# ch4r10t33r/zigz

Hardware: AMD Instinct MI355X
Metric: trace steps/sec proved (BabyBear, 2^20 RV64I trace) (higher is better)
Workload: dtype u32

## Files before the change

### zigz_amd/csrc/api_commit.cpp

```cpp
#include "api_internal.hpp"

using namespace zk;

static void caps_for(zigz_ctx *ctx, size_t npad, unsigned rn, unsigned gn) {
    ListCaps &c = ctx->caps;
    if (c.npad == npad && c.rn == rn && c.gn == gn) return;
    c.npad = npad;
    c.rn = rn;
    c.gn = gn;
    c.g_slabs = false;
    c.g_drops = c.g_skip = c.g_kept = 0;
    memset(c.r_last, 0, sizeof(c.r_last));
    memset(c.g_last, 0, sizeof(c.g_last));
    c.last_dropped = false;
    const LevelLists rw = runs_lists(npad, rn ? rn : 1), gw = cons_lists(npad);
    for (unsigned l = 0; l < RUN_MAX_LEVELS; l++) {
        c.r[l] = l <= rw.top ? (rw.cap[l] / 8 > 256 ? rw.cap[l] / 8 : 256) : 0;
        c.g[l] = l <= gw.top ? 256 : 0;
    }
}

zigz_status build_trees(zigz_ctx *ctx, const uint32_t *d_vals, size_t val_stride, size_t n_values, size_t npad,
                               uint8_t *d_slab, size_t ncols, bool record, TreeRef *ref) {
    const unsigned height = log2_floor(npad);
// ... 165 lines not shown
            if (keep) CHK(ws_get(ctx, WS_CONSMETA, kept + (upper_here ? upper_bytes : 0), &mw));
            else mw = (uint8_t *)w + ((key_bytes + idx_bytes + list_bytes + 64 + 63) & ~(size_t)63);
            b.g_rep = (uint32_t *)mw;
            t.g_rep = b.g_rep;
            t.g_store = (uint8_t *)mw + 2 * npad * 4;
            if (upper_here) t.upper = (uint8_t *)mw + kept;
            if (ctx->cons_table != w || ctx->cons_table_bytes != ctx->ws_bytes[WS_CONS] || ctx->cons_gen + RUN_MAX_LEVELS + 1 >= 4096) {
                HIPCHK(ctx, hipMemsetAsync(w, 0, key_bytes, ctx->stream));
                ctx->cons_table = w;
                ctx->cons_table_bytes = ctx->ws_bytes[WS_CONS];
                ctx->cons_gen = 1;
            }
            b.g_gen = ctx->cons_gen;
            ctx->cons_gen += top + 1;
            b.g_ctr = g_ctr;
            b.g_has_slabs = whole || ctx->caps.g_slabs;
            static const bool always_probe = getenv("ZIGZ_CONS_PROBE_ALWAYS") != nullptr;
            b.g_no_probe = ref && ctx->caps.npad == npad && ctx->caps.g_kept >= 2 && !ctx->cons_always && !always_probe;
            t.g_ncols = G.n;
            t.g_dropped = g_ctr + 8;
            for (unsigned k = 0; k < G.n; k++) t.g_j_of_col[G.c[k]] = (signed char)k;
            if (virt)
                for (unsigned k = 0; k < GS.n; k++) t.g_sd_mask |= 1ull << GS.c[k];
            ctx->build_cons_hinted = G.n;
            ctx->build_cons_levels_nodes = level_nodes;
            ctx->build_cons_sd = GS.n;
        }
        if (!t.upper) {
            void *u;
            CHK(ws_get(ctx, WS_OUT64, upper_bytes, &u));
            t.upper = (uint8_t *)u;
        }
        b.t = t;
        if (ctx->debug_skip != 2) {
            launch_runs_structure(b, ctx->stream, R.n ? stamp(4, 0) : nullptr);
            launch_cons_structure(b, ctx->stream, G.n ? stamp(4, 0) : nullptr);
        }
        if (GS.n && b.g_has_slabs) {
            const ColMap gs = slab_map(GS);
            launch_keccak_small_l01(d_vals, val_stride, n_values, npad, t.slab, stride, GS, ctx->d_sd_tables, ctx->d_sd_fallbacks + 1,
                                    (uint32_t *)sd_todo + sd_todo_words(npad, H.n), ctx->stream, stamp(3, 0), !virt, g_ctr + 8,
                                    &gs);
        }
    }
    if (ref) *ref = t;
    unsigned first_top = 0;
    if (lists) {
        for (unsigned l = 0; l <= top; l++) {
            size_t expect = 0;
            if (ref && ctx->caps.npad == npad && (ctx->caps.r_last[l] || ctx->caps.g_last[l])) {
                auto more = [](unsigned v) { return (size_t)RUN_SUBS * (v + v / 4 + 8); };
                expect = (R.n ? more(ctx->caps.r_last[l]) : 0) + (G.n ? more(ctx->caps.g_last[l]) * G.n : 0) +
                         (G.n && ctx->caps.last_dropped ? (size_t)G.n * (npad >> l) : 0);
            }
            if (ctx->debug_skip != 1) launch_level_hash(b, l, ctx->stream, stamp(5, 0), expect);
            if (l == top) break;
            ColMap m{};
            for (size_t c = 0; c < ncols; c++) {
                const int kd = kind(c);
                if (kd == 0 || (kd == 1 && l >= 1)) m.c[m.n++] = (uint8_t)c;
            }
            if (m.n) {
                const ColMap ms = slab_map(m);
                launch_keccak_level(t.slab, stride, tree_level_offset(npad, l), tree_level_offset(npad, l + 1), npad >> (l + 1), ncols,
                                    ctx->stream, stamp(keccak_level_is_wide(npad >> (l + 1), m.n) ? 1 : 2, (uint64_t)m.n * (npad >> (l + 1))), &ms);
            }
        }
        first_top = top;
    } else {
        for (unsigned l = 0; l < height; l++) {
            const size_t n_out = npad >> (l + 1);
            first_top = l;
            if (n_out <= 256) break;
            ColMap m{};
            const ColMap *pm = nullptr;
            size_t nc = ncols;
            if (H.n && l < 1) {
                for (size_t c = 0; c < ncols; c++)
                    if (kind(c) == 0) m.c[m.n++] = (uint8_t)c;
                if (m.n == 0) continue;
                pm = &m;
                nc = m.n;
            }
            launch_keccak_level(t.slab, stride, tree_level_offset(npad, l), tree_level_offset(npad, l + 1), n_out, ncols, ctx->stream,
                                stamp(keccak_level_is_wide(n_out, nc) ? 1 : 2, (uint64_t)nc * n_out), pm);
        }
    }
    if (height) {
// ... 321 lines not shown
    b.rcols = R;
    b.gcols = G;
    if (R.n) {
        t.bitmap = (unsigned long long *)(a0 + o_bitmap);
        t.prev = (unsigned short *)(a0 + o_prev);
        t.woff = (unsigned short *)(a0 + o_woff);
        t.ubase = (uint32_t *)(a0 + o_ubase);
        t.r_store = a0 + o_rstore;
        b.r_list = (uint32_t *)(a0 + o_rlist);
        b.r_stage = a0 + o_rstage;
        b.r_ctr = (unsigned long long *)(a0 + o_rctr);
    }
    if (G.n) {
        t.slab = a0 + o_slab;
        t.g_rep = (const uint32_t *)(a0 + o_grep);
        t.g_store = a0 + o_gstore;
        t.g_dropped = (const unsigned long long *)(a0 + o_gctr) + 8;
        b.g_keys = (unsigned long long *)(a0 + o_keys);
        b.g_idx = (uint32_t *)(a0 + o_idx);
        b.g_list = (uint32_t *)(a0 + o_glist);
        b.g_rep = (uint32_t *)(a0 + o_grep);
        b.g_ctr = (unsigned long long *)(a0 + o_gctr);
        b.g_has_slabs = 1;
        b.g_gen = ctx->batch_gen;
        ctx->batch_gen += t.top + 1;
    }
    b.t = t;
    set_zstride(b, S, nz);
    t = b.t;
    ColSrcs cs{};
    for (unsigned z = 0; z < nz; z++) cs.p[z] = srcs[z];
    launch_gather_cols(cs, nz, nc, N, src_stride, (uint32_t *)(a0 + o_cols), stride, S, ctx->stream);
    launch_zero_counters(nullptr, R.n ? b.r_ctr : nullptr, G.n ? b.g_ctr : nullptr, ctx->stream, nz, S);
    if (ctx->debug_skip != 2) {
        launch_runs_structure(b, ctx->stream, nullptr);
        launch_cons_structure(b, ctx->stream, nullptr);
    }
    for (unsigned l = 0; l <= t.top; l++)
        if (ctx->debug_skip != 1) launch_level_hash(b, l, ctx->stream, nullptr);
    if (height && ctx->debug_skip != 1) launch_merkle_top(t, t.top, height, nc, ctx->stream, nullptr);
    HIPCHK(ctx, hipGetLastError());
    job->tree = t;
    job->d_cols = (const uint32_t *)(a0 + o_cols);
    job->col_stride = stride;
    job->zstride = S;
    job->off_r_ctr = o_rctr;
    job->off_g_ctr = o_gctr;
    job->whole = false;
    const DoneFlag done = done_flag(ctx, 0);
    job->roots_seq = done.seq;
    launch_job_summary(t, height, ctx->h_roots, nc, R.n ? b.r_ctr : nullptr, nullptr, G.n ? b.g_ctr : nullptr, ctx->stream, done);
    HIPCHK(ctx, hipGetLastError());
    HIPCHK(ctx, hipEventRecord(job->built, ctx->stream));
    uint64_t level_nodes = 0;
    for (unsigned l = 0; l <= t.top; l++) level_nodes += npad >> l;
    job->run_cols = R.n;
    job->run_dense = (uint64_t)R.n * level_nodes;
    job->sd_cols = 0;
    job->cons_hinted = G.n;
    job->cons_levels_nodes = level_nodes;
    job->cons_sd = 0;
    job->perms0 = (uint64_t)nc * (2 * N - 1);
    job->no_eval_skip = ctx->debug_skip == 2;
    return ZIGZ_OK;
}

extern "C" zigz_status zigz_commit_begin_batch(zigz_ctx *ctx, const uint32_t *const *d_cols, size_t nproofs, size_t ncols,
                                               size_t col_stride, size_t nv, zigz_commit_job **out) {
    ZIGZ_ENTER(ctx);
    if (!ctx || !d_cols || !out || ncols == 0 || nproofs == 0 || nproofs > BATCH_MAX || nv > 40) return ZIGZ_ERR_INVALID_ARGUMENT;
    if (ncols * nproofs > ROOTS_MAX_COLS || col_stride < ((size_t)1 << nv)) return ZIGZ_ERR_INVALID_ARGUMENT;
    for (size_t z = 0; z < nproofs; z++)
// ... 302 lines not shown
```

### zigz_amd/csrc/kernels.hpp

```cpp
#pragma once
#include <hip/hip_runtime.h>
#include <stddef.h>
#include <stdint.h>

namespace zk {

struct KTime {
    hipEvent_t start, stop;
};

inline size_t tree_level_offset(size_t npad, unsigned level) { return 2 * npad - 2 * (npad >> level); }
inline size_t tree_nodes(size_t npad) { return 2 * npad; }

void launch_narrow_u64(const uint64_t *d_in, uint32_t *d_out, size_t n, uint32_t *d_flag, hipStream_t s);
void launch_reduce_u64(const uint64_t *d_in, uint32_t *d_out, size_t n, hipStream_t s);
void launch_witness_rows(const uint64_t *d_rows, size_t num_steps, size_t npad, uint32_t *d_cols, size_t stride,
                         hipStream_t s);
void launch_widen_u32(const uint32_t *d_in, uint64_t *d_out, size_t n, hipStream_t s);
struct TraceStep {
    uint64_t pc, rd_value, mem_addr, mem_value;
    int64_t imm;
    uint8_t opcode, rd, rs1, rs2, funct3, funct7, wr_reg, mem_is_read;
};
static_assert(sizeof(TraceStep) == 48, "TraceStep must mirror zigz_trace_step (48 bytes)");
// ... 155 lines not shown
LevelLists runs_lists(size_t npad, size_t ncols, const unsigned *cap_in = nullptr);
LevelLists cons_lists(size_t npad, const unsigned *cap_in = nullptr);
size_t runs_units(size_t npad, size_t ncols, unsigned long long ubase_off[RUN_MAX_LEVELS]);
size_t runs_stage_scratch_bytes(size_t npad, size_t ncols);

struct MerkleBuild {
    ZPtr<const uint32_t> vals;
    size_t val_stride, n_values, npad;
    TreeRef t;
    ColMap rcols;
    ZPtr<uint32_t> r_list;
    ZPtr<unsigned long long> r_ctr;
    ZPtr<uint8_t> r_stage;
    ColMap gcols;
    ColMap gcols_sd;
    int g_has_slabs;
    int g_no_probe;
    ZPtr<unsigned long long> g_keys;
    ZPtr<uint32_t> g_idx;
    ZPtr<uint32_t> g_rep;
    ZPtr<uint32_t> g_list;
    ZPtr<unsigned long long> g_ctr;
    unsigned g_gen;
};
inline void set_zstride(MerkleBuild &b, size_t zs, unsigned nz) {
    TreeRef &t = b.t;
    t.zstride = zs;
    t.nz = nz;
    t.slab.zs = t.upper.zs = t.bitmap.zs = t.prev.zs = t.woff.zs = t.ubase.zs = t.r_store.zs = t.g_rep.zs = t.g_store.zs = t.g_dropped.zs = zs;
    b.vals.zs = b.r_list.zs = b.r_ctr.zs = b.r_stage.zs = b.g_keys.zs = b.g_idx.zs = b.g_rep.zs = b.g_list.zs = b.g_ctr.zs = zs;
}
void launch_runs_structure(const MerkleBuild &b, hipStream_t s, const KTime *kt = nullptr);
void launch_cons_structure(const MerkleBuild &b, hipStream_t s, const KTime *kt = nullptr);
void launch_level_hash(const MerkleBuild &b, unsigned L, hipStream_t s, const KTime *kt = nullptr, size_t expect = 0);
void launch_fill_virtual(const MerkleBuild &b, hipStream_t s);
void launch_merkle_top(const TreeRef &t, unsigned first_level, unsigned height, size_t ncols, hipStream_t s, const KTime *kt = nullptr);
void launch_keccak_leaves(const uint32_t *d_vals, size_t val_stride, size_t n_values, size_t npad,
                          uint8_t *d_tree, size_t tree_stride_nodes, size_t ncols, hipStream_t s, const KTime *kt = nullptr,
                          const ColMap *cols = nullptr, const ColMap *slabs = nullptr);
void launch_keccak_level(uint8_t *d_tree, size_t tree_stride_nodes, size_t in_off, size_t out_off, size_t n_out,
                         size_t ncols, hipStream_t s, const KTime *kt = nullptr, const ColMap *slabs = nullptr);
constexpr unsigned SD_DOMAIN = 128;
constexpr size_t SD_TABLE_BYTES = (size_t)(SD_DOMAIN + SD_DOMAIN * SD_DOMAIN) * 32;
void launch_sd_tables(uint8_t *d_tables, hipStream_t s);
inline size_t sd_todo_words(size_t npad, size_t ncols) { return 2 * ncols * ((npad / 2 + 63) / 64) + 2; }
void launch_keccak_small_l01(const uint32_t *d_vals, size_t val_stride, size_t n_values, size_t npad, uint8_t *d_tree,
                             size_t tree_stride_nodes, const ColMap &cols, const uint8_t *d_tables,
                             unsigned long long *d_todo_count, uint32_t *d_todo, hipStream_t s, const KTime *kt = nullptr,
                             bool write_leaves = true, const unsigned long long *d_only_if = nullptr,
                             const ColMap *slabs = nullptr);
bool keccak_level_is_wide(size_t n_out, size_t ncols);
struct DoneFlag {
    unsigned *count = nullptr;
    unsigned long long *flag = nullptr;
    unsigned long long seq = 0;
};
void launch_publish_u64(unsigned long long *d_src, size_t n, unsigned long long *h_dst, bool rezero, hipStream_t s, DoneFlag done);
void launch_publish_u32(const uint32_t *d_src, size_t n, uint32_t *h_dst, hipStream_t s, DoneFlag done);
void launch_paths(const TreeRef &t, size_t n_values, unsigned height, const uint32_t *d_vals, size_t val_stride,
                  const uint64_t *d_idx, uint8_t *d_sib, uint8_t *d_dirs, uint32_t *d_leaf, size_t ncols, hipStream_t s,
                  DoneFlag done = DoneFlag());
TreeRef slab_tree_ref(uint8_t *d_tree, size_t npad);
void launch_gather_nodes(const uint8_t *d_tree, size_t tree_stride_nodes, size_t node, uint8_t *d_out, size_t ncols,
                         hipStream_t s);
constexpr unsigned JOB_SUMMARY_WORDS = 8 + 2 * RUN_MAX_LEVELS;
void launch_zero_counters(unsigned long long *d_sd_ctr, unsigned long long *d_r_ctr, unsigned long long *d_g_ctr, hipStream_t s,
                          unsigned nz = 0, size_t zstride = 0);
// ... 109 lines not shown
```

### zigz_amd/csrc/merkle_levels.hip

```cpp
#include "kernels.hpp"
#include "tree_dev.hpp"

namespace zk {

#ifndef ZK_CONS_TPB
#define ZK_CONS_TPB 256
#endif
constexpr int CONS_TPB = ZK_CONS_TPB;

static unsigned log2u(size_t n) { unsigned l = 0; while (((size_t)1 << l) < n) l++; return l; }

static size_t stage_fv_bytes(size_t npad, size_t ncols, unsigned s) { return ncols * (npad >> (s * RUN_STAGE_LEVELS)) * 4; }
static size_t stage_inner_bytes(size_t npad, size_t ncols, unsigned s) {
    const size_t n = npad >> (s * RUN_STAGE_LEVELS);
    return ncols * ((n + 63) / 64) * 8;
}
static size_t stage_off(size_t npad, size_t ncols, unsigned s) {
    size_t off = 0;
    for (unsigned t = 1; t < s; t++) off += stage_fv_bytes(npad, ncols, t) + stage_inner_bytes(npad, ncols, t);
    return off;
}
size_t runs_stage_scratch_bytes(size_t npad, size_t ncols) {
    const unsigned top = run_top_level(npad);
    size_t b = 64;
// ... 57 lines not shown
    x = (x | (x >> 1)) & 0x3333333333333333ull;
    x = (x | (x >> 2)) & 0x0f0f0f0f0f0f0f0full;
    x = (x | (x >> 4)) & 0x00ff00ff00ff00ffull;
    x = (x | (x >> 8)) & 0x0000ffff0000ffffull;
    x = (x | (x >> 16)) & 0x00000000ffffffffull;
    return x;
}

template <int CTRL, int ROW_MASK, int BANK_MASK>
__device__ __forceinline__ int dpp_i32(int old, int v) { return __builtin_amdgcn_update_dpp(old, v, CTRL, ROW_MASK, BANK_MASK, false); }
__device__ __forceinline__ unsigned wave_scan_add(unsigned v) {
    int s = (int)v;
    s += dpp_i32<0x111, 0xf, 0xf>(0, s);
    s += dpp_i32<0x112, 0xf, 0xf>(0, s);
    s += dpp_i32<0x114, 0xf, 0xf>(0, s);
    s += dpp_i32<0x118, 0xf, 0xf>(0, s);
    s += dpp_i32<0x142, 0xa, 0xf>(0, s);
    s += dpp_i32<0x143, 0xc, 0xf>(0, s);
    return (unsigned)s;
}
__device__ __forceinline__ int wave_scan_max(int v) {
    int s = v, t;
    t = dpp_i32<0x111, 0xf, 0xf>(-1, s); s = s > t ? s : t;
    t = dpp_i32<0x112, 0xf, 0xf>(-1, s); s = s > t ? s : t;
    t = dpp_i32<0x114, 0xf, 0xf>(-1, s); s = s > t ? s : t;
    t = dpp_i32<0x118, 0xf, 0xf>(-1, s); s = s > t ? s : t;
    t = dpp_i32<0x142, 0xa, 0xf>(-1, s); s = s > t ? s : t;
    t = dpp_i32<0x143, 0xc, 0xf>(-1, s); s = s > t ? s : t;
    return s;
}

constexpr int RUNS_WAVES = TPB / 64;
template <bool STAGE0>
__global__ __launch_bounds__(TPB) void k_runs_stage(MerkleBuild b, unsigned stage, unsigned seg_log2, unsigned rmax, unsigned nseg,
                                                    size_t in_off , size_t out_off ) {
    ZK_PRIO_SMALL();
    const unsigned lane = threadIdx.x & 63, wave = threadIdx.x >> 6;
    const unsigned y = blockIdx.y, segi = blockIdx.x * RUNS_WAVES + wave;
    if (segi >= nseg) return;
    const unsigned seg = 1u << seg_log2, words = seg / 64;
    const unsigned l_in = stage * RUN_STAGE_LEVELS;
    const size_t n_in = b.npad >> l_in;
    const size_t first = (size_t)segi * seg;
    unsigned long long E = 0, I = 0;
    uint32_t fv_mine = 0;
    {
        const uint32_t *src;
        size_t limit;
        if (STAGE0) {
            src = b.vals + (size_t)b.rcols.c[y] * b.val_stride + first;
            limit = b.n_values > first ? b.n_values - first : 0;
        } else {
            src = reinterpret_cast<const uint32_t *>(b.r_stage + in_off) + (size_t)y * n_in + first;
            limit = seg;
            const unsigned long long *inner = reinterpret_cast<const unsigned long long *>(
                b.r_stage + in_off + (size_t)b.rcols.n * n_in * 4) + ((size_t)y * n_in + first) / 64;
            if (lane < words) I = inner[lane];
        }
        uint32_t prev_last = 0;
        for (unsigned q0 = 0; q0 < words; q0 += 32) {
            uint32_t x[32];
#pragma unroll
            for (unsigned j = 0; j < 32; j++) {
                const unsigned i = (q0 + j) * 64 + lane;
                x[j] = (q0 + j < words && i < limit) ? src[i] : 0u;
            }
#pragma unroll
            for (unsigned j = 0; j < 32; j++) {
                const unsigned q = q0 + j;
                uint32_t left = (uint32_t)__builtin_amdgcn_update_dpp(0, (int)x[j], 0x138 , 0xf, 0xf, false);
                if (lane == 0) left = prev_last;
// ... 60 lines not shown
                                    ((size_t)y * n_out) / 64 + segi;
        fv[lane] = fv_mine;
        if (lane == 0) *inner = I;
    }
    unsigned my_slot = 0, my_room = 0;
    if (lane <= rmax && (STAGE0 || lane != 0)) {
        const unsigned l_abs = l_in + lane;
        const unsigned sub = (y * nseg + segi) % RUN_SUBS;
        const unsigned cap = b.t.r_lists.cap[l_abs];
        const unsigned long long pos = atomicAdd(&b.r_ctr[run_ctr_index(l_abs, sub)], (unsigned long long)my_tot);
        if (pos + my_tot > cap) atomicOr(&b.r_ctr[10], 1ull);
        my_room = pos >= cap ? 0u : (unsigned)(cap - pos < my_tot ? cap - pos : my_tot);
        my_slot = sub * cap + (unsigned)(pos < cap ? pos : cap);
        b.t.ubase[b.t.ubase_off[l_abs] + (size_t)y * nseg + segi] = my_slot;
    }
#pragma unroll
    for (unsigned r = 0; r <= RUN_STAGE_LEVELS; r++) {
        if (r > rmax || (!STAGE0 && r == 0)) continue;
        const unsigned slot0 = __shfl(my_slot, r), room = __shfl(my_room, r);
        uint32_t *list = b.r_list + b.t.r_lists.base[l_in + r];
        const size_t node0 = first >> r;
        const unsigned wr = words >> r;
        for (unsigned q = 0; q < wr; q++) {
            const unsigned lo = (unsigned)__builtin_amdgcn_readlane((int)(unsigned)need_r[r], q);
            const unsigned hi = (unsigned)__builtin_amdgcn_readlane((int)(unsigned)(need_r[r] >> 32), q);
            if ((lo | hi) == 0) continue;
            const unsigned o = (unsigned)__builtin_amdgcn_readlane((int)off_r[r], q);
            const unsigned long long m = ((unsigned long long)hi << 32) | lo;
            const unsigned at = o + __builtin_amdgcn_mbcnt_hi(hi, __builtin_amdgcn_mbcnt_lo(lo, 0));
            if (((m >> lane) & 1) && at < room) list[slot0 + at] = ((uint32_t)y << RUN_NODE_BITS) | (uint32_t)(node0 + q * 64 + lane);
        }
    }
}

void launch_runs_structure(const MerkleBuild &b, hipStream_t s, const KTime *kt) {
    if (b.rcols.n == 0) return;
    const unsigned top = b.t.r_lists.top;
    unsigned nstages = 1;
    while (nstages * RUN_STAGE_LEVELS < top) nstages++;
    for (unsigned st = 0; st < nstages; st++) {
        const size_t n_in = b.npad >> (st * RUN_STAGE_LEVELS);
        const size_t seg = n_in < RUN_SEG ? n_in : RUN_SEG;
        const unsigned rmax = top - st * RUN_STAGE_LEVELS < RUN_STAGE_LEVELS ? top - st * RUN_STAGE_LEVELS : RUN_STAGE_LEVELS;
        const bool has_next = st + 1 < nstages;
        const size_t in_off = st ? stage_off(b.npad, b.rcols.n, st) : 0;
        const size_t out_off = has_next ? stage_off(b.npad, b.rcols.n, st + 1) : ~(size_t)0;
        const unsigned nseg = (unsigned)(n_in / seg);
        const dim3 grid((nseg + RUNS_WAVES - 1) / RUNS_WAVES, b.rcols.n, b.t.nz ? b.t.nz : 1);
        hipEvent_t e0 = kt && st == 0 ? kt->start : nullptr, e1 = kt && st + 1 == nstages ? kt->stop : nullptr;
        if (st == 0) {
            if (e0 || e1) hipExtLaunchKernelGGL(k_runs_stage<true>, grid, dim3(TPB), 0, s, e0, e1, 0, b, st, log2u(seg), rmax, nseg, in_off, out_off);
            else hipLaunchKernelGGL(k_runs_stage<true>, grid, dim3(TPB), 0, s, b, st, log2u(seg), rmax, nseg, in_off, out_off);
        } else {
            if (e0 || e1) hipExtLaunchKernelGGL(k_runs_stage<false>, grid, dim3(TPB), 0, s, e0, e1, 0, b, st, log2u(seg), rmax, nseg, in_off, out_off);
            else hipLaunchKernelGGL(k_runs_stage<false>, grid, dim3(TPB), 0, s, b, st, log2u(seg), rmax, nseg, in_off, out_off);
        }
    }
}

constexpr unsigned CONS_GEN_SHIFT = 52;
__device__ __forceinline__ unsigned long long cons_mix(unsigned long long x) {
    x ^= x >> 30; x *= 0xbf58476d1ce4e5b9ull;
    x ^= x >> 27; x *= 0x94d049bb133111ebull;
    return x ^ (x >> 31);
}
constexpr unsigned CONS_TUP = 16;
__device__ __forceinline__ unsigned long long cons_leaf_payload(const MerkleBuild &b, size_t k, uint32_t *tup = nullptr) {
    unsigned long long h = 0x243f6a8885a308d3ull;
    if (tup && b.gcols.n <= CONS_TUP) {
#pragma unroll
        for (unsigned j = 0; j < CONS_TUP; j++) {
            tup[j] = (j < b.gcols.n && k < b.n_values) ? b.vals[(size_t)b.gcols.c[j] * b.val_stride + k] : 0u;
            if (j < b.gcols.n) h = cons_mix(h ^ tup[j]);
        }
    } else {
        for (unsigned j = 0; j < b.gcols.n; j++)
            h = cons_mix(h ^ (k < b.n_values ? b.vals[(size_t)b.gcols.c[j] * b.val_stride + k] : 0u));
    }
    return h & ((1ull << CONS_GEN_SHIFT) - 1);
}
__device__ __forceinline__ unsigned wave_leader(unsigned long long key, bool valid, unsigned lane) {
    unsigned long long pend = __ballot(valid);
    unsigned mine = lane;
    while (pend) {
        const unsigned ld = (unsigned)__builtin_ctzll(pend);
        const unsigned long long kk = __shfl(key, ld);
        const bool same = valid && key == kk;
        if (same) mine = ld;
// ... 39 lines not shown
}
__device__ __forceinline__ uint32_t cons_lookup(const unsigned long long *keys, const uint32_t *idx, size_t mask, unsigned long long key) {
    size_t slot = cons_mix(key) & mask;
    for (size_t tries = 0; tries <= mask; tries++) {
        if (keys[slot] == key) return idx[slot];
        slot = (slot + 1) & mask;
    }
    return 0xffffffffu;
}
constexpr unsigned CONS_SET = 2 * CONS_TPB;
__device__ __forceinline__ bool wg_first(unsigned long long *set, unsigned long long key) {
    unsigned slot = (unsigned)(cons_mix(key) >> 40) & (CONS_SET - 1);
    for (;;) {
        const unsigned long long old = atomicCAS(&set[slot], 0ull, key);
        if (old == 0) return true;
        if (old == key) return false;
        slot = (slot + 1) & (CONS_SET - 1);
    }
}
__device__ __forceinline__ void cons_insert_level(const MerkleBuild &b, unsigned long long *s_set, unsigned l, unsigned long long key,
                                                  bool elected, uint32_t node, unsigned lane, size_t wave_global) {
    const size_t mask = 2 * b.npad - 1;
    size_t where = 0;
    const unsigned g = b.g_gen + l;
    const bool won = elected && wg_first(s_set, key) && cons_insert(b.g_keys, mask, key, g, l ? g - 1 : g, &where);
    const unsigned slot = cons_take_slot(b, l, won, lane, wave_global);
    if (won) {
        b.g_list[b.t.g_lists.base[l] + slot] = node;
        b.g_idx[where] = slot;
    }
}

constexpr unsigned CONS_SAMPLE = 16;
__global__ __launch_bounds__(CONS_TPB) void k_cons_leaf_insert(MerkleBuild b, int sample) {
    ZK_PRIO_SMALL();
    __shared__ unsigned long long s_set[CONS_SET];
    if (!sample && b.g_ctr[8]) return;
    for (unsigned i = threadIdx.x; i < CONS_SET; i += CONS_TPB) s_set[i] = 0;
    __syncthreads();
    const size_t k = (size_t)blockIdx.x * CONS_TPB + threadIdx.x;
    if (sample && ((k / 64) % CONS_SAMPLE) != 0) return;
    const unsigned lane = threadIdx.x & 63;
    const bool valid = k < b.npad;
    const unsigned long long key = ((unsigned long long)b.g_gen << CONS_GEN_SHIFT) | (valid ? cons_leaf_payload(b, k) : 0);
    const unsigned ld = wave_leader(key, valid, lane);
    cons_insert_level(b, s_set, 0, key, valid && ld == lane, (uint32_t)k, lane, k / 64);
}

template <bool LEAF>
__global__ __launch_bounds__(CONS_TPB) void k_cons_pass(MerkleBuild b, unsigned lr, int do_insert) {
    ZK_PRIO_SMALL();
    __shared__ unsigned long long s_set[CONS_SET];
    if (b.g_ctr[8]) return;
    for (unsigned i = threadIdx.x; i < CONS_SET; i += CONS_TPB) s_set[i] = 0;
    __syncthreads();
    const size_t n = b.npad >> lr, c = (size_t)blockIdx.x * CONS_TPB + threadIdx.x;
    const unsigned lane = threadIdx.x & 63;
    const bool valid = c < n;
    const size_t mask = 2 * b.npad - 1;
    const unsigned g_r = b.g_gen + lr;
    const size_t off = 2 * b.npad - 2 * n;
    const size_t off_in = LEAF ? 0 : 2 * b.npad - 2 * (b.npad >> (lr - 1));
    unsigned long long key = (unsigned long long)g_r << CONS_GEN_SHIFT;
    uint32_t tup[CONS_TUP];
    if (valid) {
        if (LEAF) key |= cons_leaf_payload(b, c, tup);
        else {
            const uint2 p = *reinterpret_cast<const uint2 *>(b.g_rep + off_in + 2 * c);
            key |= ((unsigned long long)p.x << RUN_NODE_BITS) | p.y;
        }
    }
    const unsigned ld = wave_leader(key, valid, lane);
    uint32_t r = 0xffffffffu;
    if (valid && ld == lane) r = cons_lookup(b.g_keys, b.g_idx, mask, key);
    r = __shfl(r, ld);
    bool alone = false;
    if (LEAF && valid && r != 0xffffffffu) {
        const size_t rn = b.g_list[b.t.g_lists.base[0] + r];
        if (rn != c) {
            if (b.gcols.n <= CONS_TUP) {
#pragma unroll
                for (unsigned j = 0; j < CONS_TUP; j++)
                    if (j < b.gcols.n && tup[j] != (rn < b.n_values ? b.vals[(size_t)b.gcols.c[j] * b.val_stride + rn] : 0u)) alone = true;
            } else {
                for (unsigned j = 0; j < b.gcols.n; j++) {
                    const uint32_t *v = b.vals + (size_t)b.gcols.c[j] * b.val_stride;
                    if ((c < b.n_values ? v[c] : 0u) != (rn < b.n_values ? v[rn] : 0u)) { alone = true; break; }
                }
            }
        }
    }
    if (valid && r == 0xffffffffu) alone = true;
    const unsigned own = cons_take_slot(b, lr, alone, lane, c / 64);
    if (alone) {
        r = own;
        b.g_list[b.t.g_lists.base[lr] + own] = (uint32_t)c;
    }
    if (valid) b.g_rep[off + c] = r;
    if (do_insert) {
        const uint32_t r_hi = __shfl_down(r, 1);
        const bool mine = valid && !(c & 1);
        const unsigned long long k2 = ((unsigned long long)(g_r + 1) << CONS_GEN_SHIFT) | ((unsigned long long)r << RUN_NODE_BITS) | r_hi;
        const unsigned ld2 = wave_leader(k2, mine, lane);
        cons_insert_level(b, s_set, lr + 1, k2, mine && ld2 == lane, (uint32_t)(c >> 1), lane, c / 128);
    }
}

__global__ __launch_bounds__(64) void k_cons_decide(MerkleBuild b, int sample) {
    ZK_PRIO_SMALL();
    unsigned long long c = threadIdx.x < RUN_SUBS ? b.g_ctr[run_ctr_index(0, threadIdx.x)] : 0;
#pragma unroll
    for (int off = 32; off > 0; off >>= 1) c += __shfl_down(c, off);
    if (threadIdx.x == 0) {
        if (sample) {
            const bool drop = c > b.npad / CONS_SAMPLE / 4;
            b.g_ctr[8] = drop ? 1 : 0;
            b.g_ctr[9] = drop ? c * CONS_SAMPLE : 0;
        } else if (!b.g_ctr[8]) {
            b.g_ctr[9] = c;
            b.g_ctr[8] = c > b.npad / 4 ? 1 : 0;
        }
        if (!sample && b.g_ctr[8] && !b.g_has_slabs) atomicOr(&b.g_ctr[10], 2ull);
    }
}

void launch_cons_structure(const MerkleBuild &b, hipStream_t s, const KTime *kt) {
    if (b.gcols.n == 0) return;
    const unsigned top = b.t.g_lists.top;
    const unsigned nz = b.t.nz ? b.t.nz : 1;
    const dim3 g0((unsigned)((b.npad + CONS_TPB - 1) / CONS_TPB), 1, nz);
    const bool probe = b.npad >= ((size_t)1 << 16) && !b.g_no_probe;
    if (probe) {
        if (kt) hipExtLaunchKernelGGL(k_cons_leaf_insert, g0, dim3(CONS_TPB), 0, s, kt->start, nullptr, 0, b, 1);
        else hipLaunchKernelGGL(k_cons_leaf_insert, g0, dim3(CONS_TPB), 0, s, b, 1);
        hipLaunchKernelGGL(k_cons_decide, dim3(1, 1, nz), dim3(64), 0, s, b, 1);
    }
    if (kt && !probe) hipExtLaunchKernelGGL(k_cons_leaf_insert, g0, dim3(CONS_TPB), 0, s, kt->start, nullptr, 0, b, 0);
    else hipLaunchKernelGGL(k_cons_leaf_insert, g0, dim3(CONS_TPB), 0, s, b, 0);
    hipLaunchKernelGGL(k_cons_pass<true>, g0, dim3(CONS_TPB), 0, s, b, 0u, top >= 1 ? 1 : 0);
    hipLaunchKernelGGL(k_cons_decide, dim3(1, 1, nz), dim3(64), 0, s, b, 0);
    for (unsigned lr = 1; lr <= top; lr++) {
        const dim3 g((unsigned)(((b.npad >> lr) + CONS_TPB - 1) / CONS_TPB), 1, nz);
        const int ins = lr < top ? 1 : 0;
        if (kt && lr == top) hipExtLaunchKernelGGL(k_cons_pass<false>, g, dim3(CONS_TPB), 0, s, nullptr, kt->stop, 0, b, lr, ins);
        else hipLaunchKernelGGL(k_cons_pass<false>, g, dim3(CONS_TPB), 0, s, b, lr, ins);
    }
}

#ifndef ZK_LEVEL_HASH_MIN_WAVES
#define ZK_LEVEL_HASH_MIN_WAVES 1
#endif
template <bool LEAF, bool PAUSE>
__global__ __launch_bounds__(TPB, ZK_LEVEL_HASH_MIN_WAVES) void k_level_hash(MerkleBuild b, unsigned L, ColMap gdense, int prio) {
    __shared__ unsigned long long s_r[RUN_SUBS + 1], s_g[RUN_SUBS + 1];
#ifdef ZK_LEVEL_HASH_LDS_PAD
    __shared__ unsigned s_pad[ZK_LEVEL_HASH_LDS_PAD / 4];
    if (b.npad == 3) s_pad[threadIdx.x] = L;
#endif
    if (prio) ZK_PRIO_SMALL();
    const unsigned lane = threadIdx.x & 63, wave = threadIdx.x >> 6;
    const bool dropped = b.gcols.n != 0 && b.g_ctr[8] != 0;
    if (wave < 2) {
        const bool use = wave == 0 ? b.rcols.n != 0 : (b.gcols.n != 0 && !dropped);
        const unsigned long long *ctr = wave == 0 ? b.r_ctr : b.g_ctr;
        const unsigned cap = wave == 0 ? b.t.r_lists.cap[L] : b.t.g_lists.cap[L];
        unsigned long long c = use && lane < RUN_SUBS ? ctr[run_ctr_index(L, lane)] : 0;
        if (c > cap) c = cap;
        unsigned long long incl = c;
#pragma unroll
        for (int off = 1; off < 64; off <<= 1) {
            const unsigned long long a = __shfl_up(incl, off);
            if (lane >= (unsigned)off) incl += a;
        }
        unsigned long long *dst = wave == 0 ? s_r : s_g;
        if (lane < RUN_SUBS) dst[lane] = incl - c;
        if (lane == RUN_SUBS - 1) dst[RUN_SUBS] = incl;
    }
    __syncthreads();
    const size_t n_L = uniform64(b.npad >> L);
    const unsigned n_L_log2 = (unsigned)__builtin_ctzll(n_L);
    const unsigned gn = b.gcols.n;
    const size_t cR = uniform64(s_r[RUN_SUBS]), cG = uniform64(s_g[RUN_SUBS]) * gn,
                 cD = (dropped && b.g_has_slabs) ? (size_t)gdense.n * n_L : 0;
    if (blockIdx.x == 0 && threadIdx.x == 0) {
        if (cR) atomicAdd(&b.r_ctr[0], (unsigned long long)cR);
        if (cG) atomicAdd(&b.g_ctr[0], (unsigned long long)cG);
    }
    const size_t total = cR + cG + cD;
    const RLevel rl = r_level(b.t, L, true), rc = r_level(b.t, LEAF ? 0 : L - 1, true);
    const size_t r_cap = uniform64(b.t.r_lists.cap[L]), g_cap = uniform64(b.t.g_lists.cap[L]);
    const size_t g_base = uniform64(b.t.g_lists.base[L]), g_base_c = uniform64(b.t.g_lists.base[LEAF ? 0 : L - 1]);
    const size_t g_rep_c = slab_level_offset(b.npad, LEAF ? 0 : L - 1);
    const unsigned g_magic = gn > 1 ? (unsigned)(0x100000000ull / gn) : 0xffffffffu;
#pragma unroll 1
    for (size_t e = (size_t)blockIdx.x * TPB + threadIdx.x; e < total; e += (size_t)gridDim.x * TPB) {
        size_t col, k;
        uint8_t *out;
        const uint8_t *in0 = nullptr, *in1 = nullptr;
#ifdef ZK_LH_FAKE
        if (ZK_LH_FAKE) {
            col = 0;
            k = e;
            out = b.t.upper + (e & 4095) * 32;
            in0 = b.t.upper + ((2 * e) & 4095) * 32;
            in1 = in0 + 32;
        } else
#endif
        if (e < cR) {
            unsigned sub = 0;
#pragma unroll
            for (unsigned step = RUN_SUBS / 2; step; step >>= 1)
                if (s_r[sub + step] <= e) sub += step;
            const size_t slot = (size_t)sub * r_cap + (e - s_r[sub]);
            const uint32_t ent = b.r_list[rl.list_base + slot];
            const unsigned y = ent >> RUN_NODE_BITS;
            col = b.rcols.c[y];
            k = ent & ((1u << RUN_NODE_BITS) - 1);
            out = r_slot_ptr(b.t, rl, slot);
            if (!LEAF) {
                size_t c0, c1;
                r_slot_pair(b.t, rc, y, 2 * k, &c0, &c1);
                in0 = r_slot_ptr(b.t, rc, c0);
                in1 = r_slot_ptr(b.t, rc, c1);
            }
        } else if (e < cR + cG) {
            const unsigned t32 = (unsigned)(e - cR);
            unsigned ei = __umulhi(t32, g_magic), j = t32 - ei * gn;
            if (j >= gn) {
                ei++;
                j -= gn;
            }
            col = b.gcols.c[j];
            unsigned sub = 0;
#pragma unroll
            for (unsigned step = RUN_SUBS / 2; step; step >>= 1)
                if (s_g[sub + step] <= ei) sub += step;
            const size_t slot = (size_t)sub * g_cap + (ei - s_g[sub]);
            k = b.g_list[g_base + slot];
            out = b.t.g_store + ((g_base + slot) * gn + j) * 32;
            if (!LEAF) {
                const uint2 p = *reinterpret_cast<const uint2 *>(b.g_rep + g_rep_c + 2 * k);
                in0 = b.t.g_store + ((g_base_c + p.x) * gn + j) * 32;
                in1 = b.t.g_store + ((g_base_c + p.y) * gn + j) * 32;
            }
        } else {
            const size_t t = e - cR - cG;
            col = gdense.c[t >> n_L_log2];
            k = t & (n_L - 1);
            out = slab_ptr(b.t, col, L, k);
            if (!LEAF) {
                in0 = slab_ptr(b.t, col, L - 1, 2 * k);
                in1 = in0 + 32;
            }
        }
        Digest d;
        if (LEAF) d = sha3_leaf<PAUSE>((uint64_t)(k < b.n_values ? b.vals[col * b.val_stride + k] : 0u));
        else d = sha3_node<PAUSE>(load_digest_at(in0), load_digest_at(in1));
        store_digest_at(out, d);
    }
}

void launch_level_hash(const MerkleBuild &b, unsigned L, hipStream_t s, const KTime *kt, size_t expect) {
    if (b.rcols.n == 0 && b.gcols.n == 0) return;
    ColMap gd{};
    for (unsigned j = 0; j < b.gcols.n; j++) {
        bool sd = false;
        for (unsigned i = 0; i < b.gcols_sd.n; i++) sd |= b.gcols_sd.c[i] == b.gcols.c[j];
        if (L >= 2 || !sd) gd.c[gd.n++] = b.gcols.c[j];
    }
    const size_t n_L = b.npad >> L;
    size_t wgs = ((size_t)(b.rcols.n + b.gcols.n) * n_L + TPB - 1) / TPB;
    if (wgs > 2048) wgs = 2048;
#ifndef ZK_LH_GRID_BY_NODES
    {
        size_t room = (b.rcols.n ? (size_t)RUN_SUBS * b.t.r_lists.cap[L] : 0) + (b.gcols.n ? (size_t)RUN_SUBS * b.t.g_lists.cap[L] * b.gcols.n : 0);
        if (expect && expect < room) room = expect;
        size_t w2 = (room + TPB - 1) / TPB;
        if (w2 < 8) w2 = 8;
        if (w2 < wgs) wgs = w2;
    }
#endif
    const bool small = (size_t)(b.rcols.n + b.gcols.n) * n_L <= (size_t)256 * 4 * 2 * 64;
    const unsigned nz = b.t.nz ? b.t.nz : 1;
    if (nz > 1 && wgs > (2048 + nz - 1) / nz) wgs = (2048 + nz - 1) / nz;
    const bool pause = !small || (size_t)nz * (b.rcols.n + b.gcols.n) * n_L > (size_t)256 * 4 * 2 * 64;
#ifndef ZK_LH_PRIO_WGS
#define ZK_LH_PRIO_WGS 768
#endif
    const int prio = (size_t)wgs * nz <= ZK_LH_PRIO_WGS ? 1 : 0;
#ifndef ZK_LH_BIG_LDS
#define ZK_LH_BIG_LDS 28672
#endif
    const unsigned lds = prio ? 0u : (unsigned)ZK_LH_BIG_LDS;
    if (L == 0) ZK_LAUNCH(kt, (k_level_hash<true, true>), dim3((unsigned)wgs, 1, nz), dim3(TPB), lds, s, b, L, gd, prio);
    else if (!pause) ZK_LAUNCH(kt, (k_level_hash<false, false>), dim3((unsigned)wgs, 1, nz), dim3(TPB), lds, s, b, L, gd, prio);
    else ZK_LAUNCH(kt, (k_level_hash<false, true>), dim3((unsigned)wgs, 1, nz), dim3(TPB), lds, s, b, L, gd, prio);
}

__global__ __launch_bounds__(TPB) void k_merkle_top(TreeRef t, unsigned first_level, unsigned height) {
    ZK_PRIO_SMALL();
    __shared__ Digest s_d[TPB];
    const size_t col = blockIdx.y;
    for (unsigned l = first_level; l < height; l++) {
        const size_t n_out = t.npad >> (l + 1);
        Digest d;
        if (threadIdx.x < n_out) {
            Digest a, c;
            if (l == first_level) {
                a = load_digest_at(node_ptr(t, col, l, 2 * threadIdx.x));
                c = load_digest_at(node_ptr(t, col, l, 2 * threadIdx.x + 1));
            } else {
                a = s_d[2 * threadIdx.x];
                c = s_d[2 * threadIdx.x + 1];
            }
            d = sha3_node<false>(a, c);
            store_digest_at(t.lists ? upper_ptr(t, col, l + 1, threadIdx.x) : slab_ptr(t, col, l + 1, threadIdx.x), d);
        }
        __syncthreads();
        if (threadIdx.x < n_out) s_d[threadIdx.x] = d;
        __syncthreads();
    }
}
void launch_merkle_top(const TreeRef &t, unsigned first_level, unsigned height, size_t ncols, hipStream_t s, const KTime *kt) {
    ZK_LAUNCH(kt, k_merkle_top, dim3(1, (unsigned)ncols, t.nz ? t.nz : 1), dim3(TPB), 0, s, t, first_level, height);
}

// ... 27 lines not shown
```

Before: 2.198 billion.

## Fuse structure-discovery stages into combined launches and ride later passes on level hashing

Turns the runs-stage, consecutive-insert and consecutive-pass kernels into device functions. A combined k_structure kernel dispatches runs stages 0 and 1 together with the first consecutive passes, partitioned by block index. Later consecutive passes and runs stages are appended as extra workgroups to each level-hash launch, so structure work overlaps with hashing and fewer kernels are launched. In exchange, the level-hash kernels become heterogeneous and may take more LDS. The hashing now depends on the structure work for the next level running within the same grid, and that ordering is easy to get wrong.

Measured after the change: 2.286 billion, median of 6. 1.04x the previous value.

```diff
diff --git a/zigz_amd/csrc/api_commit.cpp b/zigz_amd/csrc/api_commit.cpp
--- a/zigz_amd/csrc/api_commit.cpp
+++ b/zigz_amd/csrc/api_commit.cpp
@@ -221,10 +221,7 @@
             t.upper = (uint8_t *)u;
         }
         b.t = t;
-        if (ctx->debug_skip != 2) {
-            launch_runs_structure(b, ctx->stream, R.n ? stamp(4, 0) : nullptr);
-            launch_cons_structure(b, ctx->stream, G.n ? stamp(4, 0) : nullptr);
-        }
+        if (ctx->debug_skip != 2) launch_structure(b, ctx->stream, ctx->debug_skip == 0, stamp(4, 0));
         if (GS.n && b.g_has_slabs) {
             const ColMap gs = slab_map(GS);
             launch_keccak_small_l01(d_vals, val_stride, n_values, npad, t.slab, stride, GS, ctx->d_sd_tables, ctx->d_sd_fallbacks + 1,
@@ -242,7 +239,7 @@
                 expect = (R.n ? more(ctx->caps.r_last[l]) : 0) + (G.n ? more(ctx->caps.g_last[l]) * G.n : 0) +
                          (G.n && ctx->caps.last_dropped ? (size_t)G.n * (npad >> l) : 0);
             }
-            if (ctx->debug_skip != 1) launch_level_hash(b, l, ctx->stream, stamp(5, 0), expect);
+            if (ctx->debug_skip != 1) launch_level_hash(b, l, ctx->stream, stamp(5, 0), expect, ctx->debug_skip == 0);
             if (l == top) break;
             ColMap m{};
             for (size_t c = 0; c < ncols; c++) {
@@ -630,12 +627,9 @@
     for (unsigned z = 0; z < nz; z++) cs.p[z] = srcs[z];
     launch_gather_cols(cs, nz, nc, N, src_stride, (uint32_t *)(a0 + o_cols), stride, S, ctx->stream);
     launch_zero_counters(nullptr, R.n ? b.r_ctr : nullptr, G.n ? b.g_ctr : nullptr, ctx->stream, nz, S);
-    if (ctx->debug_skip != 2) {
-        launch_runs_structure(b, ctx->stream, nullptr);
-        launch_cons_structure(b, ctx->stream, nullptr);
-    }
+    if (ctx->debug_skip != 2) launch_structure(b, ctx->stream, ctx->debug_skip == 0);
     for (unsigned l = 0; l <= t.top; l++)
-        if (ctx->debug_skip != 1) launch_level_hash(b, l, ctx->stream, nullptr);
+        if (ctx->debug_skip != 1) launch_level_hash(b, l, ctx->stream, nullptr, 0, ctx->debug_skip == 0);
     if (height && ctx->debug_skip != 1) launch_merkle_top(t, t.top, height, nc, ctx->stream, nullptr);
     HIPCHK(ctx, hipGetLastError());
     job->tree = t;
diff --git a/zigz_amd/csrc/kernels.hpp b/zigz_amd/csrc/kernels.hpp
--- a/zigz_amd/csrc/kernels.hpp
+++ b/zigz_amd/csrc/kernels.hpp
@@ -211,7 +211,9 @@
 }
 void launch_runs_structure(const MerkleBuild &b, hipStream_t s, const KTime *kt = nullptr);
 void launch_cons_structure(const MerkleBuild &b, hipStream_t s, const KTime *kt = nullptr);
-void launch_level_hash(const MerkleBuild &b, unsigned L, hipStream_t s, const KTime *kt = nullptr, size_t expect = 0);
+void launch_structure(const MerkleBuild &b, hipStream_t s, bool fused, const KTime *kt = nullptr);
+void launch_level_hash(const MerkleBuild &b, unsigned L, hipStream_t s, const KTime *kt = nullptr, size_t expect = 0,
+                       bool fused = false);
 void launch_fill_virtual(const MerkleBuild &b, hipStream_t s);
 void launch_merkle_top(const TreeRef &t, unsigned first_level, unsigned height, size_t ncols, hipStream_t s, const KTime *kt = nullptr);
 void launch_keccak_leaves(const uint32_t *d_vals, size_t val_stride, size_t n_values, size_t npad,
diff --git a/zigz_amd/csrc/merkle_levels.hip b/zigz_amd/csrc/merkle_levels.hip
--- a/zigz_amd/csrc/merkle_levels.hip
+++ b/zigz_amd/csrc/merkle_levels.hip
@@ -113,11 +113,11 @@
 
 constexpr int RUNS_WAVES = TPB / 64;
 template <bool STAGE0>
-__global__ __launch_bounds__(TPB) void k_runs_stage(MerkleBuild b, unsigned stage, unsigned seg_log2, unsigned rmax, unsigned nseg,
-                                                    size_t in_off , size_t out_off ) {
+__device__ __forceinline__ void runs_stage_wg(const MerkleBuild &b, unsigned bx, unsigned y, unsigned stage, unsigned seg_log2,
+                                              unsigned rmax, unsigned nseg, size_t in_off, size_t out_off) {
     ZK_PRIO_SMALL();
     const unsigned lane = threadIdx.x & 63, wave = threadIdx.x >> 6;
-    const unsigned y = blockIdx.y, segi = blockIdx.x * RUNS_WAVES + wave;
+    const unsigned segi = bx * RUNS_WAVES + wave;
     if (segi >= nseg) return;
     const unsigned seg = 1u << seg_log2, words = seg / 64;
     const unsigned l_in = stage * RUN_STAGE_LEVELS;
@@ -244,28 +244,50 @@
         }
     }
 }
+template <bool STAGE0>
+__global__ __launch_bounds__(TPB) void k_runs_stage(MerkleBuild b, unsigned stage, unsigned seg_log2, unsigned rmax, unsigned nseg,
+                                                    size_t in_off , size_t out_off ) {
+    runs_stage_wg<STAGE0>(b, blockIdx.x, blockIdx.y, stage, seg_log2, rmax, nseg, in_off, out_off);
+}
+
+struct RunsStage {
+    unsigned stage, seg_log2, rmax, nseg, wgs;
+    size_t in_off, out_off;
+};
+static unsigned runs_nstages(const MerkleBuild &b) {
+    unsigned nstages = 1;
+    while (nstages * RUN_STAGE_LEVELS < b.t.r_lists.top) nstages++;
+    return b.rcols.n ? nstages : 0;
+}
+static RunsStage runs_stage_shape(const MerkleBuild &b, unsigned st) {
+    RunsStage r{};
+    if (st >= runs_nstages(b)) return r;
+    const unsigned top = b.t.r_lists.top;
+    const size_t n_in = b.npad >> (st * RUN_STAGE_LEVELS);
+    const size_t seg = n_in < RUN_SEG ? n_in : RUN_SEG;
+    r.stage = st;
+    r.seg_log2 = log2u(seg);
+    r.rmax = top - st * RUN_STAGE_LEVELS < RUN_STAGE_LEVELS ? top - st * RUN_STAGE_LEVELS : RUN_STAGE_LEVELS;
+    r.nseg = (unsigned)(n_in / seg);
+    r.wgs = (r.nseg + RUNS_WAVES - 1) / RUNS_WAVES;
+    r.in_off = st ? stage_off(b.npad, b.rcols.n, st) : 0;
+    r.out_off = st + 1 < runs_nstages(b) ? stage_off(b.npad, b.rcols.n, st + 1) : ~(size_t)0;
+    return r;
+}
 
 void launch_runs_structure(const MerkleBuild &b, hipStream_t s, const KTime *kt) {
     if (b.rcols.n == 0) return;
-    const unsigned top = b.t.r_lists.top;
-    unsigned nstages = 1;
-    while (nstages * RUN_STAGE_LEVELS < top) nstages++;
+    const unsigned nstages = runs_nstages(b);
     for (unsigned st = 0; st < nstages; st++) {
-        const size_t n_in = b.npad >> (st * RUN_STAGE_LEVELS);
-        const size_t seg = n_in < RUN_SEG ? n_in : RUN_SEG;
-        const unsigned rmax = top - st * RUN_STAGE_LEVELS < RUN_STAGE_LEVELS ? top - st * RUN_STAGE_LEVELS : RUN_STAGE_LEVELS;
-        const bool has_next = st + 1 < nstages;
-        const size_t in_off = st ? stage_off(b.npad, b.rcols.n, st) : 0;
-        const size_t out_off = has_next ? stage_off(b.npad, b.rcols.n, st + 1) : ~(size_t)0;
-        const unsigned nseg = (unsigned)(n_in / seg);
-        const dim3 grid((nseg + RUNS_WAVES - 1) / RUNS_WAVES, b.rcols.n, b.t.nz ? b.t.nz : 1);
+        const RunsStage r = runs_stage_shape(b, st);
+        const dim3 grid(r.wgs, b.rcols.n, b.t.nz ? b.t.nz : 1);
         hipEvent_t e0 = kt && st == 0 ? kt->start : nullptr, e1 = kt && st + 1 == nstages ? kt->stop : nullptr;
         if (st == 0) {
-            if (e0 || e1) hipExtLaunchKernelGGL(k_runs_stage<true>, grid, dim3(TPB), 0, s, e0, e1, 0, b, st, log2u(seg), rmax, nseg, in_off, out_off);
-            else hipLaunchKernelGGL(k_runs_stage<true>, grid, dim3(TPB), 0, s, b, st, log2u(seg), rmax, nseg, in_off, out_off);
+            if (e0 || e1) hipExtLaunchKernelGGL(k_runs_stage<true>, grid, dim3(TPB), 0, s, e0, e1, 0, b, st, r.seg_log2, r.rmax, r.nseg, r.in_off, r.out_off);
+            else hipLaunchKernelGGL(k_runs_stage<true>, grid, dim3(TPB), 0, s, b, st, r.seg_log2, r.rmax, r.nseg, r.in_off, r.out_off);
         } else {
-            if (e0 || e1) hipExtLaunchKernelGGL(k_runs_stage<false>, grid, dim3(TPB), 0, s, e0, e1, 0, b, st, log2u(seg), rmax, nseg, in_off, out_off);
-            else hipLaunchKernelGGL(k_runs_stage<false>, grid, dim3(TPB), 0, s, b, st, log2u(seg), rmax, nseg, in_off, out_off);
+            if (e0 || e1) hipExtLaunchKernelGGL(k_runs_stage<false>, grid, dim3(TPB), 0, s, e0, e1, 0, b, st, r.seg_log2, r.rmax, r.nseg, r.in_off, r.out_off);
+            else hipLaunchKernelGGL(k_runs_stage<false>, grid, dim3(TPB), 0, s, b, st, r.seg_log2, r.rmax, r.nseg, r.in_off, r.out_off);
         }
     }
 }
@@ -371,13 +393,12 @@
 }
 
 constexpr unsigned CONS_SAMPLE = 16;
-__global__ __launch_bounds__(CONS_TPB) void k_cons_leaf_insert(MerkleBuild b, int sample) {
+__device__ __forceinline__ void cons_leaf_insert_wg(const MerkleBuild &b, int sample, unsigned bx, unsigned long long *s_set) {
     ZK_PRIO_SMALL();
-    __shared__ unsigned long long s_set[CONS_SET];
     if (!sample && b.g_ctr[8]) return;
     for (unsigned i = threadIdx.x; i < CONS_SET; i += CONS_TPB) s_set[i] = 0;
     __syncthreads();
-    const size_t k = (size_t)blockIdx.x * CONS_TPB + threadIdx.x;
+    const size_t k = (size_t)bx * CONS_TPB + threadIdx.x;
     if (sample && ((k / 64) % CONS_SAMPLE) != 0) return;
     const unsigned lane = threadIdx.x & 63;
     const bool valid = k < b.npad;
@@ -385,15 +406,18 @@
     const unsigned ld = wave_leader(key, valid, lane);
     cons_insert_level(b, s_set, 0, key, valid && ld == lane, (uint32_t)k, lane, k / 64);
 }
+__global__ __launch_bounds__(CONS_TPB) void k_cons_leaf_insert(MerkleBuild b, int sample) {
+    __shared__ unsigned long long s_set[CONS_SET];
+    cons_leaf_insert_wg(b, sample, blockIdx.x, s_set);
+}
 
 template <bool LEAF>
-__global__ __launch_bounds__(CONS_TPB) void k_cons_pass(MerkleBuild b, unsigned lr, int do_insert) {
+__device__ __forceinline__ void cons_pass_wg(const MerkleBuild &b, unsigned lr, int do_insert, unsigned bx, unsigned long long *s_set) {
     ZK_PRIO_SMALL();
-    __shared__ unsigned long long s_set[CONS_SET];
     if (b.g_ctr[8]) return;
     for (unsigned i = threadIdx.x; i < CONS_SET; i += CONS_TPB) s_set[i] = 0;
     __syncthreads();
-    const size_t n = b.npad >> lr, c = (size_t)blockIdx.x * CONS_TPB + threadIdx.x;
+    const size_t n = b.npad >> lr, c = (size_t)bx * CONS_TPB + threadIdx.x;
     const unsigned lane = threadIdx.x & 63;
     const bool valid = c < n;
     const size_t mask = 2 * b.npad - 1;
@@ -444,6 +468,11 @@
         cons_insert_level(b, s_set, lr + 1, k2, mine && ld2 == lane, (uint32_t)(c >> 1), lane, c / 128);
     }
 }
+template <bool LEAF>
+__global__ __launch_bounds__(CONS_TPB) void k_cons_pass(MerkleBuild b, unsigned lr, int do_insert) {
+    __shared__ unsigned long long s_set[CONS_SET];
+    cons_pass_wg<LEAF>(b, lr, do_insert, blockIdx.x, s_set);
+}
 
 __global__ __launch_bounds__(64) void k_cons_decide(MerkleBuild b, int sample) {
     ZK_PRIO_SMALL();
@@ -463,12 +492,14 @@
     }
 }
 
+static bool cons_probe(const MerkleBuild &b) { return b.npad >= ((size_t)1 << 16) && !b.g_no_probe; }
+
 void launch_cons_structure(const MerkleBuild &b, hipStream_t s, const KTime *kt) {
     if (b.gcols.n == 0) return;
     const unsigned top = b.t.g_lists.top;
     const unsigned nz = b.t.nz ? b.t.nz : 1;
     const dim3 g0((unsigned)((b.npad + CONS_TPB - 1) / CONS_TPB), 1, nz);
-    const bool probe = b.npad >= ((size_t)1 << 16) && !b.g_no_probe;
+    const bool probe = cons_probe(b);
     if (probe) {
         if (kt) hipExtLaunchKernelGGL(k_cons_leaf_insert, g0, dim3(CONS_TPB), 0, s, kt->start, nullptr, 0, b, 1);
         else hipLaunchKernelGGL(k_cons_leaf_insert, g0, dim3(CONS_TPB), 0, s, b, 1);
@@ -490,7 +521,7 @@
 #define ZK_LEVEL_HASH_MIN_WAVES 1
 #endif
 template <bool LEAF, bool PAUSE>
-__global__ __launch_bounds__(TPB, ZK_LEVEL_HASH_MIN_WAVES) void k_level_hash(MerkleBuild b, unsigned L, ColMap gdense, int prio) {
+__device__ __forceinline__ void level_hash_wg(const MerkleBuild &b, unsigned L, const ColMap &gdense, int prio, unsigned bx, unsigned nbx) {
     __shared__ unsigned long long s_r[RUN_SUBS + 1], s_g[RUN_SUBS + 1];
 #ifdef ZK_LEVEL_HASH_LDS_PAD
     __shared__ unsigned s_pad[ZK_LEVEL_HASH_LDS_PAD / 4];
@@ -521,7 +552,7 @@
     const unsigned gn = b.gcols.n;
     const size_t cR = uniform64(s_r[RUN_SUBS]), cG = uniform64(s_g[RUN_SUBS]) * gn,
                  cD = (dropped && b.g_has_slabs) ? (size_t)gdense.n * n_L : 0;
-    if (blockIdx.x == 0 && threadIdx.x == 0) {
+    if (bx == 0 && threadIdx.x == 0) {
         if (cR) atomicAdd(&b.r_ctr[0], (unsigned long long)cR);
         if (cG) atomicAdd(&b.g_ctr[0], (unsigned long long)cG);
     }
@@ -532,7 +563,7 @@
     const size_t g_rep_c = slab_level_offset(b.npad, LEAF ? 0 : L - 1);
     const unsigned g_magic = gn > 1 ? (unsigned)(0x100000000ull / gn) : 0xffffffffu;
 #pragma unroll 1
-    for (size_t e = (size_t)blockIdx.x * TPB + threadIdx.x; e < total; e += (size_t)gridDim.x * TPB) {
+    for (size_t e = (size_t)bx * TPB + threadIdx.x; e < total; e += (size_t)nbx * TPB) {
         size_t col, k;
         uint8_t *out;
         const uint8_t *in0 = nullptr, *in1 = nullptr;
@@ -598,8 +629,84 @@
         store_digest_at(out, d);
     }
 }
-
-void launch_level_hash(const MerkleBuild &b, unsigned L, hipStream_t s, const KTime *kt, size_t expect) {
+template <bool LEAF, bool PAUSE>
+__global__ __launch_bounds__(TPB, ZK_LEVEL_HASH_MIN_WAVES) void k_level_hash(MerkleBuild b, unsigned L, ColMap gdense, int prio) {
+    level_hash_wg<LEAF, PAUSE>(b, L, gdense, prio, blockIdx.x, gridDim.x);
+}
+
+#ifndef ZK_STRUCT_SEPARATE
+static_assert(CONS_TPB == TPB, "the fused structure launches share the 256-thread workgroups of the hash and runs kernels "
+                               "(build with -DZK_STRUCT_SEPARATE for another ZK_CONS_TPB)");
+template <bool FIRST>
+__global__ __launch_bounds__(TPB) void k_structure(MerkleBuild b, unsigned nruns, RunsStage rs) {
+    __shared__ unsigned long long s_set[CONS_SET];
+    if (blockIdx.x < nruns) {
+        runs_stage_wg<FIRST>(b, blockIdx.x % rs.wgs, blockIdx.x / rs.wgs, rs.stage, rs.seg_log2, rs.rmax, rs.nseg, rs.in_off, rs.out_off);
+        return;
+    }
+    const unsigned w = blockIdx.x - nruns;
+    if (FIRST) cons_leaf_insert_wg(b, 0, w, s_set);
+    else cons_pass_wg<true>(b, 0u, b.t.g_lists.top >= 1 ? 1 : 0, w, s_set);
+}
+static_assert((RUN_NODE_BITS - 8 + RUN_STAGE_LEVELS - 1) / RUN_STAGE_LEVELS <= 3, "a runs stage would ride above level 0");
+template <bool LEAF, bool PAUSE, bool STAGE>
+__global__ __launch_bounds__(TPB, ZK_LEVEL_HASH_MIN_WAVES) void k_level_hash_rides(MerkleBuild b, unsigned L, ColMap gdense, int prio,
+                                                                                   unsigned npass, RunsStage rs) {
+    extern __shared__ unsigned long long s_dyn[];
+    if (blockIdx.x < npass) {
+        cons_pass_wg<false>(b, L + 1, L + 1 < b.t.g_lists.top ? 1 : 0, blockIdx.x, s_dyn);
+        return;
+    }
+    const unsigned w = blockIdx.x - npass, nrs = STAGE ? rs.wgs * b.rcols.n : 0;
+    if (STAGE && w < nrs) {
+        runs_stage_wg<false>(b, w % rs.wgs, w / rs.wgs, rs.stage, rs.seg_log2, rs.rmax, rs.nseg, rs.in_off, rs.out_off);
+        return;
+    }
+    level_hash_wg<LEAF, PAUSE>(b, L, gdense, prio, w - nrs, gridDim.x - npass - nrs);
+}
+#endif
+
+#define ZK_LAUNCH_EV(e0, e1, kern, grid, block, lds, s, ...)                                                      \
+    do {                                                                                                          \
+        const hipEvent_t ev0_ = (e0), ev1_ = (e1);                                                                \
+        if (ev0_ || ev1_) hipExtLaunchKernelGGL(kern, grid, block, lds, s, ev0_, ev1_, 0, __VA_ARGS__);           \
+        else hipLaunchKernelGGL(kern, grid, block, lds, s, __VA_ARGS__);                                          \
+    } while (0)
+
+static RunsStage runs_stage_riding(const MerkleBuild &b, unsigned L) { return runs_stage_shape(b, L + 2); }
+
+void launch_structure(const MerkleBuild &b, hipStream_t s, bool fused, const KTime *kt) {
+#ifdef ZK_STRUCT_SEPARATE
+    fused = false;
+#endif
+    if (!fused) {
+        KTime k0{kt ? kt->start : nullptr, nullptr}, k1{nullptr, kt ? kt->stop : nullptr};
+        if (!b.gcols.n) k0.stop = k1.stop;
+        if (!b.rcols.n) k1.start = k0.start;
+        launch_runs_structure(b, s, kt ? &k0 : nullptr);
+        launch_cons_structure(b, s, kt ? &k1 : nullptr);
+        return;
+    }
+#ifndef ZK_STRUCT_SEPARATE
+    const unsigned nz = b.t.nz ? b.t.nz : 1;
+    const unsigned ncons = b.gcols.n ? (unsigned)((b.npad + CONS_TPB - 1) / CONS_TPB) : 0;
+    const RunsStage r0 = runs_stage_shape(b, 0), r1 = runs_stage_shape(b, 1);
+    const unsigned nra = r0.wgs * b.rcols.n, nrb = r1.wgs * b.rcols.n, na = nra + ncons, nb = nrb + ncons;
+    if (!na) return;
+    hipEvent_t e0 = kt ? kt->start : nullptr;
+    const hipEvent_t stop = kt ? kt->stop : nullptr;
+    if (ncons && cons_probe(b)) {
+        ZK_LAUNCH_EV(e0, nullptr, k_cons_leaf_insert, dim3(ncons, 1, nz), dim3(CONS_TPB), 0, s, b, 1);
+        e0 = nullptr;
+        hipLaunchKernelGGL(k_cons_decide, dim3(1, 1, nz), dim3(64), 0, s, b, 1);
+    }
+    ZK_LAUNCH_EV(e0, nb || ncons ? nullptr : stop, k_structure<true>, dim3(na, 1, nz), dim3(TPB), 0, s, b, nra, r0);
+    if (nb) ZK_LAUNCH_EV(nullptr, ncons ? nullptr : stop, k_structure<false>, dim3(nb, 1, nz), dim3(TPB), 0, s, b, nrb, r1);
+    if (ncons) ZK_LAUNCH_EV(nullptr, stop, k_cons_decide, dim3(1, 1, nz), dim3(64), 0, s, b, 0);
+#endif
+}
+
+void launch_level_hash(const MerkleBuild &b, unsigned L, hipStream_t s, const KTime *kt, size_t expect, bool fused) {
     if (b.rcols.n == 0 && b.gcols.n == 0) return;
     ColMap gd{};
     for (unsigned j = 0; j < b.gcols.n; j++) {
@@ -631,6 +738,22 @@
 #define ZK_LH_BIG_LDS 28672
 #endif
     const unsigned lds = prio ? 0u : (unsigned)ZK_LH_BIG_LDS;
+#ifndef ZK_STRUCT_SEPARATE
+    const unsigned npass = fused && b.gcols.n && L < b.t.g_lists.top ? (unsigned)(((b.npad >> (L + 1)) + CONS_TPB - 1) / CONS_TPB) : 0;
+    const RunsStage rs = fused ? runs_stage_riding(b, L) : RunsStage{};
+    const unsigned nride = npass + rs.wgs * b.rcols.n;
+    if (nride) {
+        const dim3 grid(nride + (unsigned)wgs, 1, nz);
+        const unsigned lds_r = npass && lds < CONS_SET * 8 ? CONS_SET * 8 : lds;
+        if (L == 0 && rs.wgs) ZK_LAUNCH(kt, (k_level_hash_rides<true, true, true>), grid, dim3(TPB), lds_r, s, b, L, gd, prio, npass, rs);
+        else if (L == 0) ZK_LAUNCH(kt, (k_level_hash_rides<true, true, false>), grid, dim3(TPB), lds_r, s, b, L, gd, prio, npass, rs);
+        else if (!pause) ZK_LAUNCH(kt, (k_level_hash_rides<false, false, false>), grid, dim3(TPB), lds_r, s, b, L, gd, prio, npass, rs);
+        else ZK_LAUNCH(kt, (k_level_hash_rides<false, true, false>), grid, dim3(TPB), lds_r, s, b, L, gd, prio, npass, rs);
+        return;
+    }
+#else
+    (void)fused;
+#endif
     if (L == 0) ZK_LAUNCH(kt, (k_level_hash<true, true>), dim3((unsigned)wgs, 1, nz), dim3(TPB), lds, s, b, L, gd, prio);
     else if (!pause) ZK_LAUNCH(kt, (k_level_hash<false, false>), dim3((unsigned)wgs, 1, nz), dim3(TPB), lds, s, b, L, gd, prio);
     else ZK_LAUNCH(kt, (k_level_hash<false, true>), dim3((unsigned)wgs, 1, nz), dim3(TPB), lds, s, b, L, gd, prio);
```
